# mwickert/scikit-dsp-comm

Hardware: AMD Instinct MI355X
Metric: complex64 MSamples/s (FIR-1024 tap, 2^26 samples) (higher is better)
Workload: dtype c64

## Files before the change

scikit-dsp-comm_amd/csrc/fir_ols.hip:

```cpp
#include "skdsp_internal.hpp"
#include "ols_tables.hpp"
#include "fir_route.hpp"
#include <cstdlib>
#include <cstdio>


namespace skdsp {

using namespace ols;
typedef float v4f_t __attribute__((ext_vector_type(4)));

struct OlsPlan {
    int ntaps = 0;
    int ov = 0;
    int V = 0;
    float4 *T1 = nullptr, *T2 = nullptr, *Hp = nullptr;
};

struct OlsArgs {
    const cf *x;
    cf *y;
    int64_t n, n_hist;
    const float4 *T1, *T2, *Hp;
    int ov, V, a0;
    int keep;
    int aligned;
    int64_t ntiles;
    int dec;
    unsigned dec_magic;
    int up;
    int64_t up_pitch;
    int up_sb, up_pbs, up_pb0;
    int64_t n_keep;
    const unsigned *halo_flag;
// ... 421 lines not shown
        if (DEC) {
            const unsigned j0 = r0 + (unsigned)(i + pos) * (unsigned)A.up, j1 = j0 + 64u * (unsigned)A.up;
            auto keep = [&](unsigned j, float val, bool inside) __attribute__((always_inline)) {
                const unsigned k = (unsigned)(((unsigned long long)j * A.dec_magic) >> 32);
                if (k * M == j && (int)k < qlim && inside) yq[k] = val;
            };
            keep(j0, e0.x, whole || i < lim);
            keep(j1, e1.x, whole || i + 64 < lim);
            keep(j0 + jv, e0.y, whole || i < limb);
            keep(j1 + jv, e1.y, whole || i + 64 < limb);
            continue;
        }
        char *ua = ua0 + (size_t)(a - a0) * step, *ub = ub0 + (size_t)(a - a0) * step;
        if (whole || i < lim) *reinterpret_cast<float *>(ua + b0) = e0.x;
        if (whole || i + 64 < lim) *reinterpret_cast<float *>(ua + b1) = e1.x;
        if (whole || i < limb) *reinterpret_cast<float *>(ub + b0) = e0.y;
        if (whole || i + 64 < limb) *reinterpret_cast<float *>(ub + b1) = e1.y;
    }
}


__device__ __forceinline__ OlsCareful ols_careful_args(const OlsArgs &A, int ph, bool cx)
{
    OlsCareful c;
    c.x = A.x; c.y = A.y; c.n = A.n; c.n_hist = A.n_hist; c.n_keep = A.n_keep; c.up_pitch = A.up_pitch;
    c.V = A.V; c.dec = A.dec; c.up = A.up;
    const int esz = cx ? 8 : 4;
    c.L = A.up_sb / esz;
    c.p0 = (A.up_pb0 + ph * A.up_pbs) / esz;
    c.cf = A.cf;
    return c;
}

template <bool REAL, bool DEC, bool UP = false, bool XR = false>
__global__ __launch_bounds__(256, 2) void ols_tile_kernel(OlsArgs A)
{
    __shared__ float4 lds[kLdsUnits];
    __shared__ float4 t2lds[2 * kT2Units];
    __shared__ unsigned long long ols_noted;
    if (threadIdx.x == 0) ols_noted = 0;
    constexpr int HS = (DEC && !UP) ? (REAL ? 4 : 5) : 0;
    float4 *T2f = t2lds;
    float4 *T2t = t2lds + kT2Units;
    const int t = threadIdx.x;

    {
        const float4 w = A.T2[t];
        T2f[t] = w;
        T2t[(t & 15) * 16 + (t >> 4)] = w;
    }
    cf tw[16];
#pragma unroll
    for (int k1 = 1; k1 < 16; ++k1) tw[k1] = lo(A.T1[k1 * 256 + t]);
    tw[0] = make_float2(1.f, 0.f);

    __syncthreads();
    int it = 0;
    float4 hh[16];
    int64_t tile = (gridDim.x % 8 == 0) ? (int64_t)(blockIdx.x % 8) * (gridDim.x / 8) + blockIdx.x / 8
                                                                 : (int64_t)blockIdx.x;
    const bool t0_last = A.halo_flag != nullptr;
    auto phys = [&](int64_t w) -> int64_t {
        if (UP) return (int64_t)__builtin_amdgcn_readfirstlane((unsigned)w / (unsigned)A.up);
        return t0_last ? (w + 1 < A.ntiles ? w + 1 : 0) : w;
    };
    auto phase_of = [&](int64_t w) -> int { return (int)__builtin_amdgcn_readfirstlane((unsigned)w % (unsigned)A.up); };
    if (!UP) load_H(t, A.Hp, hh);
    cf v[32];
    if (tile < A.ntiles) {
        if (t0_last && phys(tile) == 0) wait_halo(A);
        load_any<REAL, XR>(A, phys(tile), t, v);
    }
    if constexpr (XR) {
#pragma unroll
        for (int i = 0; i < 32; i += 8)
            asm volatile("" ::"v"(v[i].x), "v"(v[i + 1].x), "v"(v[i + 2].x), "v"(v[i + 3].x), "v"(v[i + 4].x), "v"(v[i + 5].x), "v"(v[i + 6].x), "v"(v[i + 7].x));
    } else {
#pragma unroll
    for (int i = 0; i < 32; i += 8)
        asm volatile("" ::"v"(v[i].x), "v"(v[i].y), "v"(v[i + 1].x), "v"(v[i + 1].y), "v"(v[i + 2].x), "v"(v[i + 2].y),
                     "v"(v[i + 3].x), "v"(v[i + 3].y), "v"(v[i + 4].x), "v"(v[i + 4].y), "v"(v[i + 5].x), "v"(v[i + 5].y),
                     "v"(v[i + 6].x), "v"(v[i + 6].y), "v"(v[i + 7].x), "v"(v[i + 7].y));
    }
    for (; tile < A.ntiles; tile += gridDim.x, ++it) {
        if (HS > 0) {
            int tt = t;
            asm volatile("" : "+v"(tt));
#pragma unroll
            for (int j = 16 - HS; j < 16; ++j) hh[j] = vld(reinterpret_cast<const volatile float4 *>(A.Hp) + (unsigned)(j * 256 + tt));
        }
        if (UP) {
            int tt = t;
            asm volatile("" : "+v"(tt));
            const volatile float4 *hp = reinterpret_cast<const volatile float4 *>(A.Hp) + (size_t)phase_of(tile) * 4096;
#pragma unroll
            for (int j = 0; j < 16; ++j) hh[j] = vld(hp + (unsigned)(j * 256 + tt));
        }
        if (REAL) fwd_pass1_real(t, v, tw, lds); else fwd_pass1(t, v, tw, lds);
        __syncthreads();
        cf Z[32];
        fwd_pass23(t, T2f, lds, Z);
        mul_H(hh, Z);
        const int64_t next = tile + gridDim.x;
        cf nx[32];
        __builtin_amdgcn_s_setprio(3);
        if (next < A.ntiles) {
            if (t0_last && phys(next) == 0) wait_halo(A);
            load_any<REAL, XR>(A, phys(next), t, nx);
        }
        __builtin_amdgcn_s_setprio(0);
        inv_pass32(t, T2t, lds, Z);
        __syncthreads();
        inv_pass1(t, tw, lds, v);
        if constexpr (XR) {
#pragma unroll
            for (int i = 0; i < 32; i += 8)
                asm volatile("" ::"v"(nx[i].x), "v"(nx[i + 1].x), "v"(nx[i + 2].x), "v"(nx[i + 3].x), "v"(nx[i + 4].x), "v"(nx[i + 5].x), "v"(nx[i + 6].x), "v"(nx[i + 7].x)
                             : "memory");
        } else {
#pragma unroll
        for (int i = 0; i < 32; i += 8)
            asm volatile("" ::"v"(nx[i].x), "v"(nx[i].y), "v"(nx[i + 1].x), "v"(nx[i + 1].y), "v"(nx[i + 2].x), "v"(nx[i + 2].y),
                         "v"(nx[i + 3].x), "v"(nx[i + 3].y), "v"(nx[i + 4].x), "v"(nx[i + 4].y), "v"(nx[i + 5].x), "v"(nx[i + 5].y),
                         "v"(nx[i + 6].x), "v"(nx[i + 6].y), "v"(nx[i + 7].x), "v"(nx[i + 7].y)
                         : "memory");
        }
        __builtin_amdgcn_s_setprio(3);
        if (UP) {
            if (!DEC && A.up_pitch) {
                OlsArgs B = A;
                B.y = REAL ? reinterpret_cast<cf *>(reinterpret_cast<float *>(A.y) + (int64_t)phase_of(tile) * A.up_pitch) : A.y + (int64_t)phase_of(tile) * A.up_pitch;
                store_any<REAL, false>(B, phys(tile), t, v, lds);
            } else if (REAL) {
                store_tile_real_up<DEC>(A, phys(tile), phase_of(tile), t, v);
            } else {
                store_tile_up<DEC>(A, phys(tile), phase_of(tile), t, v);
            }
        } else {
            store_any<REAL, DEC>(A, phys(tile), t, v, lds);
        }
        __builtin_amdgcn_s_setprio(0);
        if (__builtin_expect(__any(not_finite(v[31].x) | not_finite(v[31].y)), 0)) careful_note(&ols_noted, it);
#pragma unroll
        for (int i = 0; i < 32; ++i) v[i] = nx[i];
#ifdef SK_OLS_KEEP_B3
        __syncthreads();
#else
        if constexpr (REAL || DEC || UP || XR) __syncthreads();
#endif
    }
    const unsigned long long noted = careful_noted(&ols_noted);
    if (__builtin_expect(noted != 0, 0)) {
        int64_t w = (gridDim.x % 8 == 0) ? (int64_t)(blockIdx.x % 8) * (gridDim.x / 8) + blockIdx.x / 8 : (int64_t)blockIdx.x;
        for (int64_t k = 0; w < A.ntiles; w += gridDim.x, ++k)
            if (careful_step_noted(noted, k))
                careful_ols_tile<float, REAL, DEC, UP, XR>(ols_careful_args(A, UP ? phase_of(w) : 0, !(REAL || XR)), phys(w), UP ? phase_of(w) : 0, t);
    }
}


template <bool REAL, int MF>
__global__ __launch_bounds__(256, 2) void ols_fold_kernel(OlsArgs A)
{
    __shared__ float4 lds[kLdsUnits];
    __shared__ float4 t2lds[2 * kT2Units];
    __shared__ unsigned long long ols_noted;
    if (threadIdx.x == 0) ols_noted = 0;
    float4 *T2f = t2lds, *T2t = t2lds + kT2Units;
    const int t = threadIdx.x;
    {
        const float4 w = A.T2[t];
        T2f[t] = w;
        T2t[(t & 15) * 16 + (t >> 4)] = w;
    }
    cf tw[16];
#pragma unroll
    for (int k1 = 1; k1 < 16; ++k1) tw[k1] = lo(A.T1[k1 * 256 + t]);
    tw[0] = make_float2(1.f, 0.f);
    __syncthreads();
    float4 hh[16];
    auto first_tile = [&]() -> int64_t { return (gridDim.x % 8 == 0) ? (int64_t)(blockIdx.x % 8) * (gridDim.x / 8) + blockIdx.x / 8 : (int64_t)blockIdx.x; };
    int64_t tile = first_tile();
    load_H(t, A.Hp, hh);
    cf v[32];
    if (tile < A.ntiles) load_any<REAL, false>(A, tile, t, v);
#pragma unroll
    for (int i = 0; i < 32; i += 8)
        asm volatile("" ::"v"(v[i].x), "v"(v[i].y), "v"(v[i + 1].x), "v"(v[i + 1].y), "v"(v[i + 2].x), "v"(v[i + 2].y),
                     "v"(v[i + 3].x), "v"(v[i + 3].y), "v"(v[i + 4].x), "v"(v[i + 4].y), "v"(v[i + 5].x), "v"(v[i + 5].y),
                     "v"(v[i + 6].x), "v"(v[i + 6].y), "v"(v[i + 7].x), "v"(v[i + 7].y));
    constexpr int LS = MF / 2;
    const int b = t >> 4, q = t & 15;
    const bool active = q % LS == 0;
    const int j0 = (32 / MF) * b + q / LS;
    constexpr int JA = 512 / MF;
    for (int64_t step = 0; tile < A.ntiles; tile += gridDim.x, ++step) {
        if (REAL) fwd_pass1_real(t, v, tw, lds); else fwd_pass1(t, v, tw, lds);
        __syncthreads();
        cf Z[32];
        fwd_pass23(t, T2f, lds, Z);
        mul_H(hh, Z);
        const int64_t next = tile + gridDim.x;
        cf nx[32];
        __builtin_amdgcn_s_setprio(3);
        if (next < A.ntiles) load_any<REAL, false>(A, next, t, nx);
        __builtin_amdgcn_s_setprio(0);
        inv_pass32_fold<MF>(t, T2t, lds, Z);
        __syncthreads();
        cf o[16];
#pragma unroll
        for (int a = 0; a < 16; ++a) o[a] = make_float2(0.f, 0.f);
        inv_pass1_fold<MF>(t, tw, lds, o);
#pragma unroll
        for (int i = 0; i < 32; i += 8)
            asm volatile("" ::"v"(nx[i].x), "v"(nx[i].y), "v"(nx[i + 1].x), "v"(nx[i + 1].y), "v"(nx[i + 2].x), "v"(nx[i + 2].y),
                         "v"(nx[i + 3].x), "v"(nx[i + 3].y), "v"(nx[i + 4].x), "v"(nx[i + 4].y), "v"(nx[i + 5].x), "v"(nx[i + 5].y),
                         "v"(nx[i + 6].x), "v"(nx[i + 6].y), "v"(nx[i + 7].x), "v"(nx[i + 7].y)
                         : "memory");
// ... 90 lines not shown
            ScalarBase xc(A.x + e0);
#pragma unroll
            for (int a = 0; a < 16; ++a) {
                const v2f_t r = __builtin_nontemporal_load(xc.at<const v2f_t>(JA * 8 * a, off));
                in[a] = make_float2(r.x, r.y);
            }
        }
        return;
    }
#pragma unroll
    for (int a = 0; a < 16; ++a) {
        int64_t ia, ib;
        if (REAL) {
            const float *xr = reinterpret_cast<const float *>(A.x);
            float va = 0.f, vb = 0.f;
            if (fetch((unsigned)(JA * a + tt), ia) && ia >= -A.rep_hist && ia < A.n_in) va = xr[ia];
            if (fetch((unsigned)(JA * a + tt + VD), ib) && ib >= -A.rep_hist && ib < A.n_in) vb = xr[ib];
            in[a] = make_float2(va, vb);
        } else if (fetch((unsigned)(JA * a + tt), ia) && ia >= -A.rep_hist && ia < A.n_in) {
            in[a] = A.x[ia];
        }
    }
}

template <bool REAL, int LF>
__global__ __launch_bounds__(256, 2) void ols_rep_kernel(OlsArgs A)
{
    __shared__ float4 lds[kLdsUnits];
    __shared__ float4 t2lds[2 * kT2Units];
    __shared__ unsigned long long ols_noted;
    if (threadIdx.x == 0) ols_noted = 0;
    float4 *T2f = t2lds, *T2t = t2lds + kT2Units;
    const int t = threadIdx.x;
    {
        const float4 w = A.T2[t];
        T2f[t] = w;
        T2t[(t & 15) * 16 + (t >> 4)] = w;
    }
    cf tw[16];
#pragma unroll
    for (int k1 = 1; k1 < 16; ++k1) tw[k1] = lo(A.T1[k1 * 256 + t]);
    tw[0] = make_float2(1.f, 0.f);
    __syncthreads();
    float4 hh[16];
    auto first_tile = [&]() -> int64_t { return (gridDim.x % 8 == 0) ? (int64_t)(blockIdx.x % 8) * (gridDim.x / 8) + blockIdx.x / 8 : (int64_t)blockIdx.x; };
    int64_t tile = first_tile();
    load_H(t, A.Hp, hh);
    cf in[16];
    if (tile < A.ntiles) load_rep<REAL, LF>(A, tile, t, in);
#pragma unroll
    for (int i = 0; i < 16; i += 8)
        asm volatile("" ::"v"(in[i].x), "v"(in[i].y), "v"(in[i + 1].x), "v"(in[i + 1].y), "v"(in[i + 2].x), "v"(in[i + 2].y),
                     "v"(in[i + 3].x), "v"(in[i + 3].y), "v"(in[i + 4].x), "v"(in[i + 4].y), "v"(in[i + 5].x), "v"(in[i + 5].y),
                     "v"(in[i + 6].x), "v"(in[i + 6].y), "v"(in[i + 7].x), "v"(in[i + 7].y));
    for (int64_t step = 0; tile < A.ntiles; tile += gridDim.x, ++step) {
        fwd_pass1_rep<LF>(t, in, tw, lds);
        __syncthreads();
        cf Z[32];
        fwd_pass23_rep<LF>(t, T2f, lds, Z);
        mul_H(hh, Z);
        const int64_t next = tile + gridDim.x;
        cf nx[16];
        __builtin_amdgcn_s_setprio(3);
        if (next < A.ntiles) load_rep<REAL, LF>(A, next, t, nx);
        __builtin_amdgcn_s_setprio(0);
        inv_pass32(t, T2t, lds, Z);
        __syncthreads();
        cf v[32];
        inv_pass1(t, tw, lds, v);
#pragma unroll
        for (int i = 0; i < 16; i += 8)
            asm volatile("" ::"v"(nx[i].x), "v"(nx[i].y), "v"(nx[i + 1].x), "v"(nx[i + 1].y), "v"(nx[i + 2].x), "v"(nx[i + 2].y),
                         "v"(nx[i + 3].x), "v"(nx[i + 3].y), "v"(nx[i + 4].x), "v"(nx[i + 4].y), "v"(nx[i + 5].x), "v"(nx[i + 5].y),
                         "v"(nx[i + 6].x), "v"(nx[i + 6].y), "v"(nx[i + 7].x), "v"(nx[i + 7].y)
                         : "memory");
        __builtin_amdgcn_s_setprio(3);
        store_any<REAL, false>(A, tile, t, v, lds);
        __builtin_amdgcn_s_setprio(0);
        if (__builtin_expect(__any(not_finite(v[31].x) | not_finite(v[31].y)), 0)) careful_note(&ols_noted, step);
#pragma unroll
        for (int i = 0; i < 16; ++i) in[i] = nx[i];
        __syncthreads();
// ... 129 lines not shown
int fir_ols_launch(FirHandle *h, const void *x, int64_t n, int64_t n_hist, void *y, hipStream_t s, int dec, int reserve_wgs,
                   const unsigned *halo_flag, unsigned halo_seq, unsigned *halo_err, int halo_spins)
{
    note_path("fir_ols");
    if (n <= 0) return SKDSP_OK;
    if (dec > 1) n = (n / dec) * dec;
    if (n <= 0) return SKDSP_OK;
    SK_CHECK(fir_ols_supported(fir_shape_of(h)), SKDSP_ERR_UNSUPPORTED, "fir_ols: needs complex64 (or float32 with real taps) and 2..4097 taps");
    SK_CHECK(dec <= 32768, SKDSP_ERR_UNSUPPORTED, "fir_ols: decimation by %d (the decimating store takes M <= 32768)", dec);
    int rc = ensure_plan(h);
    if (rc) return rc;
    OlsPlan *p = h->ols;
    OlsArgs A;
    A.x = (const cf *)x;
    A.y = (cf *)y;
    A.n = n;
    A.n_hist = n_hist;
    A.T1 = p->T1; A.T2 = p->T2; A.Hp = p->Hp;
    A.ov = p->ov; A.V = p->V; A.a0 = p->ov / 512; A.keep = ols_keep_blocks(A.a0);
    const bool real = h->dtype == SKDSP_F32;
    A.aligned = ((((uintptr_t)x) | ((uintptr_t)y)) & (real ? 3 : 7)) == 0;
    int64_t ntiles = (n + p->V - 1) / p->V;
    if (real) ntiles = (ntiles + 1) / 2;
    SK_CHECK(ntiles < (int64_t)1 << 31, SKDSP_ERR_BADARG, "fir_ols: too many tiles");
    A.ntiles = ntiles;
    A.dec = dec > 1 ? dec : 1;
    A.dec_magic = A.dec > 1 ? (unsigned)((((unsigned long long)1 << 32) + A.dec - 1) / A.dec) : 0u;
    A.n_keep = n;
    A.up = 1; A.up_pitch = 0; A.up_sb = A.up_pbs = A.up_pb0 = 0;
    A.halo_flag = halo_flag; A.halo_seq = halo_seq; A.halo_err = halo_err; A.halo_spins = halo_spins > 0 ? halo_spins : (1 << 21);
    A.rep_L = 0; A.rep_lr = 1; A.rep_magic = 0; A.n_in = 0; A.rep_hist = 0;
    if ((rc = fir_careful(h, &A.cf))) return rc;
    SK_CHECK(!(halo_flag && real), SKDSP_ERR_UNSUPPORTED, "fir_ols: halo flag wait is for complex64 shards");
    int64_t grid = 2 * (int64_t)ctx().num_cus;
    if (reserve_wgs < 0) reserve_wgs = opt().ols_reserve;
    if (reserve_wgs > 0 && grid >= 4 * (int64_t)reserve_wgs) grid -= reserve_wgs;
    if (grid > ntiles) grid = ntiles;
    const int mf = A.dec % 16 == 0 ? 16 : (A.dec % 8 == 0 ? 8 : (A.dec % 4 == 0 ? 4 : (A.dec % 2 == 0 ? 2 : 1)));
    const bool fold = opt().fir_dn_fold && !halo_flag && mf > 1;
    if (fold) {
        const int mr = A.dec / mf;
        A.dec_magic = mr > 1 ? (unsigned)((((unsigned long long)1 << 32) + mr - 1) / mr) : 0u;
#define SK_FOLD(MF)                                                                                                  \
    if (real) hipLaunchKernelGGL((ols_fold_kernel<true, MF>), dim3((unsigned)grid), dim3(256), 0, s, A);             \
    else hipLaunchKernelGGL((ols_fold_kernel<false, MF>), dim3((unsigned)grid), dim3(256), 0, s, A)
        switch (mf) {
        case 2: SK_FOLD(2); break;
        case 4: SK_FOLD(4); break;
        case 8: SK_FOLD(8); break;
        default: SK_FOLD(16); break;
        }
#undef SK_FOLD
    } else if (A.dec > 1) {
        if (real) hipLaunchKernelGGL((ols_tile_kernel<true, true>), dim3((unsigned)grid), dim3(256), 0, s, A);
        else hipLaunchKernelGGL((ols_tile_kernel<false, true>), dim3((unsigned)grid), dim3(256), 0, s, A);
    } else {
        if (real) hipLaunchKernelGGL((ols_tile_kernel<true, false>), dim3((unsigned)grid), dim3(256), 0, s, A);
        else hipLaunchKernelGGL((ols_tile_kernel<false, false>), dim3((unsigned)grid), dim3(256), 0, s, A);
    }
    SK_HIP(hipGetLastError());
    return SKDSP_OK;
}


static int up_plan(FirHandle *h, int L, int kind, OlsPlan **out)
{
    const int key = kind == 1 ? -L : (kind == 2 ? 1000 + L : (kind == 3 ? 100000 + L : L));
    for (auto &u : h->ols_up)
        if (u.L == key) { *out = u.plan; return SKDSP_OK; }
    int rc = build_plan(h, L, out, kind);
// ... 5 lines not shown
static int up_walk(FirHandle *h, int kind, const void *x, int64_t n, int64_t n_hist, int L, void *y, hipStream_t s, int dec, int64_t rows_pitch)
{
    OlsPlan *p = nullptr;
    int rc = up_plan(h, L, kind, &p);
    if (rc) return rc;
    const bool xr = kind == 1;
    const bool real = h->dtype == SKDSP_F32 && !xr;
    const int cnt = kind == 1 ? L / 2 : (kind == 2 ? 1 : L);
    OlsArgs A;
    A.x = (const cf *)x;
    A.y = (cf *)y;
    A.n = n;
    A.n_hist = n_hist;
    A.T1 = p->T1; A.T2 = p->T2; A.Hp = p->Hp;
    A.ov = p->ov; A.V = p->V; A.a0 = p->ov / 512; A.keep = ols_keep_blocks(A.a0);
    const int esz = h->dtype == SKDSP_F32 ? 4 : 8;
    A.aligned = xr ? (((uintptr_t)x & 3) == 0 && ((uintptr_t)y & (L % 2 ? 3 : 7)) == 0) : ((((uintptr_t)x) | ((uintptr_t)y)) & (real ? 3 : 7)) == 0;
    int64_t ntiles = (n + p->V - 1) / p->V;
    if (real) ntiles = (ntiles + 1) / 2;
    ntiles *= cnt;
    SK_CHECK(ntiles < (int64_t)1 << 31, SKDSP_ERR_BADARG, "fir_ols_up: too many tiles");
    A.ntiles = ntiles;
    A.dec = dec;
    A.dec_magic = dec > 1 ? (unsigned)((((unsigned long long)1 << 32) + dec - 1) / dec) : 0u;
    A.n_keep = dec > 1 ? (n * L) / dec : n;
    A.up = cnt;
    A.up_pitch = dec > 1 ? 0 : rows_pitch;
    A.up_sb = L * esz;
    A.up_pbs = xr ? 8 : esz;
    A.up_pb0 = kind == 2 ? (L - 1) * esz : 0;
    A.halo_flag = nullptr; A.halo_seq = 0; A.halo_err = nullptr; A.halo_spins = 0;
    A.rep_L = 0; A.rep_lr = 1; A.rep_magic = 0; A.n_in = 0; A.rep_hist = 0;
    if ((rc = fir_careful(h, &A.cf))) return rc;
    int64_t grid = 2 * (int64_t)ctx().num_cus;
    const int reserve_wgs = opt().ols_reserve;
    if (reserve_wgs > 0 && grid >= 4 * (int64_t)reserve_wgs) grid -= reserve_wgs;
    if (grid > ntiles) grid = ntiles;
    if (xr) {
        if (L == 2 && A.up_pitch == 0) A.up_pitch = 1;
        hipLaunchKernelGGL((ols_tile_kernel<false, false, true, true>), dim3((unsigned)grid), dim3(256), 0, s, A);
    } else if (dec > 1) {
        if (real) hipLaunchKernelGGL((ols_tile_kernel<true, true, true>), dim3((unsigned)grid), dim3(256), 0, s, A);
        else hipLaunchKernelGGL((ols_tile_kernel<false, true, true>), dim3((unsigned)grid), dim3(256), 0, s, A);
    } else {
        if (real) hipLaunchKernelGGL((ols_tile_kernel<true, false, true>), dim3((unsigned)grid), dim3(256), 0, s, A);
        else hipLaunchKernelGGL((ols_tile_kernel<false, false, true>), dim3((unsigned)grid), dim3(256), 0, s, A);
    }
    SK_HIP(hipGetLastError());
    return SKDSP_OK;
}

int fir_ols_rep_launch(FirHandle *h, const void *x, int64_t n, int64_t n_hist, int L, void *y, hipStream_t s)
{
    note_path("fir_ols_rep");
    if (n <= 0) return SKDSP_OK;
    SK_CHECK(fir_ols_rep_supported(fir_shape_of(h), L, opt().fir_up_rep), SKDSP_ERR_UNSUPPORTED, "fir_ols_rep: needs complex64 (or float32 with real taps), an even L and 2..4097 taps");
    OlsPlan *p = nullptr;
    int rc = up_plan(h, L, 3, &p);
    if (rc) return rc;
    const bool real = h->dtype == SKDSP_F32;
    const int lf = L % 16 == 0 ? 16 : (L % 8 == 0 ? 8 : (L % 4 == 0 ? 4 : 2));
    OlsArgs A;
    A.x = (const cf *)x;
    A.y = (cf *)y;
    A.n = n * L;
    A.n_hist = n_hist * L;
    A.T1 = p->T1; A.T2 = p->T2; A.Hp = p->Hp;
    A.ov = p->ov; A.V = p->V; A.a0 = p->ov / 512; A.keep = ols_keep_blocks(A.a0);
    A.aligned = ((((uintptr_t)x) | ((uintptr_t)y)) & (real ? 3 : 7)) == 0;
    int64_t ntiles = (A.n + p->V - 1) / p->V;
    if (real) ntiles = (ntiles + 1) / 2;
    SK_CHECK(ntiles < (int64_t)1 << 31, SKDSP_ERR_BADARG, "fir_ols_rep: too many tiles");
    A.ntiles = ntiles;
    A.dec = 1; A.dec_magic = 0; A.n_keep = A.n;
    A.up = 1; A.up_pitch = 0; A.up_sb = A.up_pbs = A.up_pb0 = 0;
    A.halo_flag = nullptr; A.halo_seq = 0; A.halo_err = nullptr; A.halo_spins = 0;
    A.rep_L = L; A.rep_lr = L / lf;
    A.rep_magic = A.rep_lr > 1 ? (unsigned)((((unsigned long long)1 << 32) + A.rep_lr - 1) / A.rep_lr) : 0u;
    A.n_in = n; A.rep_hist = n_hist;
    if ((rc = fir_careful(h, &A.cf))) return rc;
    int64_t grid = 2 * (int64_t)ctx().num_cus;
    const int reserve_wgs = opt().ols_reserve;
    if (reserve_wgs > 0 && grid >= 4 * (int64_t)reserve_wgs) grid -= reserve_wgs;
    if (grid > ntiles) grid = ntiles;
#define SK_REP(LFV)                                                                                                  \
    if (real) hipLaunchKernelGGL((ols_rep_kernel<true, LFV>), dim3((unsigned)grid), dim3(256), 0, s, A);             \
    else hipLaunchKernelGGL((ols_rep_kernel<false, LFV>), dim3((unsigned)grid), dim3(256), 0, s, A)
    switch (lf) {
    case 2: SK_REP(2); break;
    case 4: SK_REP(4); break;
    case 8: SK_REP(8); break;
    default: SK_REP(16); break;
    }
#undef SK_REP
    SK_HIP(hipGetLastError());
    return SKDSP_OK;
}

int fir_ols_up_launch(FirHandle *h, const void *x, int64_t n, int64_t n_hist, int L, void *y, hipStream_t s, int dec, int64_t rows_pitch, int paired)
{
    note_path("fir_ols_up");
    if (n <= 0) return SKDSP_OK;
    SK_CHECK(dec >= 1 && dec <= 4096 && (dec == 1 || L <= 64), SKDSP_ERR_UNSUPPORTED, "fir_ols_up: L / M = %d / %d (the fused L / M store takes L <= 64, M <= 4096)", L, dec);
    SK_CHECK(fir_ols_up_supported(fir_shape_of(h), L), SKDSP_ERR_UNSUPPORTED, "fir_ols_up: needs complex64 (or float32 with real taps), 2 <= L <= 256, 2..4097 taps per phase");
    if (!paired) return up_walk(h, 0, x, n, n_hist, L, y, s, dec, rows_pitch);
    SK_CHECK(fir_ols_up_pairs(fir_shape_of(h), L, dec, (unsigned)(uintptr_t)y, opt().fir_up_pair) && (L % 2 == 0 || rows_pitch == 0), SKDSP_ERR_BADARG,
             "fir_ols_up: phases in pairs need float32, real taps, no decimation, and an 8-byte aligned destination (even L) or the strided form (odd L, 7 .. 13)");
    int rc = up_walk(h, 1, x, n, n_hist, L, y, s, 1, rows_pitch);
    if (rc || L % 2 == 0) return rc;
    return up_walk(h, 2, x, n, n_hist, L, y, s, 1, 0);
}

}
```

scikit-dsp-comm_amd/csrc/runtime.hip:

```cpp
#include "api_internal.hpp"
#include <cstdarg>
#include <cstdio>
#include <cstdlib>
#include <cstring>

namespace skdsp {

static thread_local char g_err[1024] = "";

void set_error(const char *fmt, ...)
{
    va_list ap;
    va_start(ap, fmt);
    vsnprintf(g_err, sizeof(g_err), fmt, ap);
    va_end(ap);
}

int hip_fail(hipError_t e, const char *what, const char *file, int line)
{
    set_error("HIP error %d (%s) in %s at %s:%d", (int)e, hipGetErrorString(e), what, file, line);
    (void)hipGetLastError();
    if (e == hipErrorOutOfMemory) return SKDSP_ERR_NOMEM;
    if (e == hipErrorNoDevice || e == hipErrorInvalidDevice) return SKDSP_ERR_NODEVICE;
    return SKDSP_ERR_HIP;
// ... 34 lines not shown
int async_err_check(Context &c)
{
    if (!c.async_err) return SKDSP_OK;
    volatile unsigned *w = c.async_err;
    if (w[kAsyncErrHalo]) {
        w[kAsyncErrHalo] = 0;
        opt().shard_two_launches = 1;
        set_error("fir_filter_shard: a sharded step since the last synchronisation gave up waiting for its halo inside the filter "
                  "launch (the first tile of that step is invalid); switched to the two-launch form (option shard_two_launches) -- "
                  "repeat the step on every rank");
        return SKDSP_ERR_RCCL;
    }
    if (w[kAsyncErrIirLookback]) {
        w[kAsyncErrIirLookback] = 0;
        set_error("iir: a look-back poll of a single-pass scan launched since the last synchronisation timed out (the results of "
                  "that call are invalid; option iir_two_pass = 1 selects the two-pass scan)");
        return SKDSP_ERR_HIP;
    }
    return SKDSP_OK;
}

int sync_checked()
{
    SK_HIP(hipStreamSynchronize(ctx().stream));
    return async_err_check(ctx());
}

namespace {
struct OptEntry { const char *name; int Options::*field; };
const OptEntry kOptTable[] = {
    {"device", &Options::device}, {"fir_algo", &Options::fir_algo}, {"dn_no_ols", &Options::dn_no_ols},
    {"fir_mm", &Options::fir_mm}, {"fir_bx", &Options::fir_bx}, 
    
    {"ols_reserve", &Options::ols_reserve}, {"fir_bx_t16", &Options::fir_bx_t16}, {"fir_bank_per", &Options::fir_bank_per}, {"ols_keep_overlap", &Options::ols_keep_overlap}, {"fir_dn_fold", &Options::fir_dn_fold}, {"fir_up_rep", &Options::fir_up_rep}, {"iir_seq", &Options::iir_seq}, {"psd_f32_image", &Options::psd_f32_image}, {"iir_up_jump", &Options::iir_up_jump}, {"iir_dn_t96", &Options::iir_dn_t96}, {"iir_up_lean", &Options::iir_up_lean}, {"iir_planar", &Options::iir_planar}, 
    {"iir_dn_full", &Options::iir_dn_full}, {"iir_no_mfma", &Options::iir_no_mfma}, 
    {"iir_two_pass", &Options::iir_two_pass}, {"iir_par", &Options::iir_par}, {"iir_par_v32", &Options::iir_par_v32}, {"iir_up_fused", &Options::iir_up_fused}, {"fir_up_ols_min", &Options::fir_up_ols_min}, {"fir_updn_fused", &Options::fir_updn_fused}, {"fir_up4k", &Options::fir_up4k}, {"fir_up4k_group", &Options::fir_up4k_group}, {"fir_up4k_staged", &Options::fir_up4k_staged}, {"fir_up2k", &Options::fir_up2k}, {"fir_dn4k", &Options::fir_dn4k}, {"fir_up_pair", &Options::fir_up_pair}, {"fir_up_rows_min", &Options::fir_up_rows_min}, {"iir_dn_compact", &Options::iir_dn_compact}, 
    {"shard_two_launches", &Options::shard_two_launches}, {"shard_probe", &Options::shard_probe}, {"shard_halo_state", &Options::shard_halo_state},
    {"shard_self_halo", &Options::shard_self_halo}, {"dist_force_comm", &Options::dist_force_comm},
    {"host_chunk_log2", &Options::host_chunk_log2}, {"host_pipeline", &Options::host_pipeline}, {"host_multi_slot", &Options::host_multi_slot},
};
int parse_opt(const char *name, const char *v)
{
    if (!strcmp(name, "fir_algo")) {
        if (!strcmp(v, "direct")) return SKDSP_FIR_DIRECT;
        if (!strcmp(v, "ols")) return SKDSP_FIR_OLS;
        if (!strcmp(v, "auto")) return SKDSP_FIR_AUTO;
    }
    if (!*v) return 1;
    return atoi(v);
}
Options options_from_env()
{
    Options o;
    for (const OptEntry &e : kOptTable) {
        char key[64] = "SKDSP_";
        size_t k = 6;
        for (const char *p = e.name; *p && k + 1 < sizeof(key); ++p) key[k++] = (char)toupper((unsigned char)*p);
        key[k] = 0;
        if (const char *v = getenv(key)) o.*(e.field) = parse_opt(e.name, v);
    }
    return o;
}
}

Options &opt()
{
    static Options o = options_from_env();
// ... 313 lines not shown
```

scikit-dsp-comm_amd/csrc/skdsp_internal.hpp:

```cpp
#pragma once
#include <hip/hip_runtime.h>
#include <stdint.h>
#include <string>
#include <vector>
#include <memory>
#include <mutex>
#include "../../include/skdsp.h"
#include "careful.hpp"

namespace skdsp {

void set_error(const char *fmt, ...);
int hip_fail(hipError_t e, const char *what, const char *file, int line);

#define SK_HIP(call)                                                        \
    do {                                                                    \
        hipError_t _e = (call);                                             \
        if (_e != hipSuccess) return skdsp::hip_fail(_e, #call, __FILE__, __LINE__); \
    } while (0)

#define SK_CHECK(cond, code, ...)            \
    do {                                     \
        if (!(cond)) {                       \
            skdsp::set_error(__VA_ARGS__);   \
            return (code);                   \
        }                                    \
    } while (0)

void note_path(const char *engine);

struct Options {
    int device = -1;
    int fir_algo = 0;
    int dn_no_ols = 0;
    int fir_mm = 1;
    int fir_bx = 1;
    int fir_bx_t16 = 1;
    int ols_keep_overlap = 1;
    int ols_reserve = 8;
    int iir_planar = 0;
    int iir_dn_full = 0;
    int iir_no_mfma = 0;
    int iir_two_pass = 0;
    int iir_par = 1;
    int iir_par_v32 = 1;
    int iir_up_jump = 1;
    int iir_seq = 1;
    int iir_up_lean = 1;
    int iir_dn_t96 = 1;
    int iir_dn_compact = 1;
    int fir_up_ols_min = 64;
    int fir_up_rows_min = -1;
    int fir_up_pair = 1;
    int fir_up4k = 1;
    int fir_up2k = 1;
    int fir_up_rep = 1;
    int fir_dn_fold = 1;
    int fir_dn4k = 1;
    int fir_up4k_group = 4;
    int fir_up4k_staged = 1;
    int fir_bank_per = 0;
    int fir_updn_fused = 1;
    int iir_up_fused = 1;
    int shard_two_launches = 0;
    int shard_probe = 1;
    int shard_halo_state = 0;
    int shard_self_halo = 0;
    int dist_force_comm = 0;
    int host_chunk_log2 = 22;
    int host_pipeline = 1;
    int psd_f32_image = 0;
    int host_multi_slot = 1;
// ... 57 lines not shown
    T *dev = nullptr;
    DevTable() = default;
    DevTable(const DevTable &) = delete;
    DevTable &operator=(const DevTable &) = delete;
    ~DevTable()
    {
        if (dev) (void)hipFree(dev);
    }
    int upload(const T *src, size_t count)
    {
        SK_HIP(hipMalloc((void **)&dev, count * sizeof(T)));
        SK_HIP(hipMemcpy(dev, src, count * sizeof(T), hipMemcpyHostToDevice));
        return SKDSP_OK;
    }
    int upload(const std::vector<T> &v) { return upload(v.data(), v.size()); }
};
struct TilePlan {
    int key = 0;
    virtual ~TilePlan() {}
};
typedef std::vector<std::unique_ptr<TilePlan>> TilePlans;
template <class P, class Fill> int tile_plan(TilePlans &plans, int key, P **out, Fill fill)
{
    for (auto &q : plans)
        if (q->key == key) { *out = static_cast<P *>(q.get()); return SKDSP_OK; }
    std::unique_ptr<P> p(new P());
    p->key = key;
    const int rc = fill(*p);
    if (rc) return rc;
    *out = p.get();
    plans.push_back(std::move(p));
    return SKDSP_OK;
}
inline int64_t persistent_grid(int64_t ntiles)
{
    int64_t grid = 2 * (int64_t)ctx().num_cus;
    const int reserve_wgs = opt().ols_reserve;
    if (reserve_wgs > 0 && grid >= 4 * (int64_t)reserve_wgs) grid -= reserve_wgs;
    return grid > ntiles ? ntiles : grid;
}
inline bool elem_aligned(const void *x, const void *y, int esz) { return ((((uintptr_t)x) | ((uintptr_t)y)) & (uintptr_t)(esz - 1)) == 0; }

struct OlsPlan;
struct Ols64Plan;
struct FirHandle : HandleBase {
    int ntaps = 0;
    bool taps_complex = false;
    int algo = SKDSP_FIR_AUTO;
    std::vector<double> taps_host;
    void *taps64_dev = nullptr;
    struct Poly { int L; int T; void *dev; };
    std::vector<Poly> poly;
    struct SwTab { int L, M, R; void *taps; void *rho; };
    std::vector<SwTab> sw;
    struct MmTab { int L, M, Lp, q, DS, RS, U0, K4; void *At; };
    std::vector<MmTab> mm;
    struct BxTab { int L, M, Lp, q, DS, RS, RT, U0, KB, RSP, KSP; float tap_inv = 0.0f; void *At = nullptr; };
    std::vector<BxTab> bx;
    OlsPlan *ols = nullptr;
    struct OlsUp { int L; OlsPlan *plan; };
    std::vector<OlsUp> ols_up;
    TilePlans up4k;
    TilePlans up2k;
    TilePlans dn4k;
    Ols64Plan *ols64 = nullptr;
    struct Ols64Up { int L; Ols64Plan *plan; };
    std::vector<Ols64Up> ols64_up;
    std::vector<FirHandle *> parts;
    int part_seg = 0;
    std::vector<FirHandle *> heads;
    ~FirHandle();
};
// ... 101 lines not shown
```

scikit-dsp-comm_amd/csrc/tile_walk.hpp:

```cpp
#pragma once
#include "ols_core.hpp"

namespace skdsp {
namespace walk {

using ols::cf;

__device__ __forceinline__ int64_t first_tile()
{
    return (gridDim.x % 8 == 0) ? (int64_t)(blockIdx.x % 8) * (gridDim.x / 8) + blockIdx.x / 8 : (int64_t)blockIdx.x;
}

__device__ __forceinline__ void twiddles_4k(int t, const float2 *T2, const float2 *tw, cf *T2f, cf *T2t, cf *twl)
{
    const cf w = T2[t];
    T2f[t] = w;
    T2t[(t & 15) * 16 + (t >> 4)] = w;
#pragma unroll
    for (int k = 0; k < 15; ++k) twl[k * 256 + t] = tw[k * 256 + t];
}

__device__ __forceinline__ float4 vld(const volatile float4 *p)
{
    float4 r;
    r.x = p->x; r.y = p->y; r.z = p->z; r.w = p->w;
    return r;
}
__device__ __forceinline__ void load_H(const float4 *Hp, int q, int t, float4 *hh)
{
    int tt = t;
    asm volatile("" : "+v"(tt));
    const volatile float4 *hp = reinterpret_cast<const volatile float4 *>(Hp) + (size_t)q * 2048;
#pragma unroll
    for (int k = 0; k < 8; ++k) hh[k] = vld(hp + (unsigned)(k * 256 + tt));
}

template <int N> __device__ __forceinline__ void pin(cf *v)
{
#pragma unroll
    for (int i = 0; i < N; i += 8)
        asm volatile("" : "+v"(v[i].x), "+v"(v[i].y), "+v"(v[i + 1].x), "+v"(v[i + 1].y), "+v"(v[i + 2].x), "+v"(v[i + 2].y), "+v"(v[i + 3].x), "+v"(v[i + 3].y),
                     "+v"(v[i + 4].x), "+v"(v[i + 4].y), "+v"(v[i + 5].x), "+v"(v[i + 5].y), "+v"(v[i + 6].x), "+v"(v[i + 6].y), "+v"(v[i + 7].x), "+v"(v[i + 7].y));
}
template <int N> __device__ __forceinline__ void settle(const float4 *hh)
// ... 25 lines not shown
```

Measured before the change: 298,600.

## Balance last-round OLS tiles across XCDs and overlap table prologue with first load

Replaces the fixed stride tile walk in the OLS tile kernel with a RoundWalk that keeps full rounds XCD-grouped but spreads the partial last round evenly across the eight XCDs. It also reorders the kernel prologue so the first input tile load is issued before twiddle, T2 and H table loads, letting that global latency overlap with table setup. Grid sizing is centralised into a helper with an optional slots override. This risks extra per-iteration index arithmetic and register pressure from holding tables alongside the first tile.

```diff
diff --git a/scikit-dsp-comm_amd/csrc/fir_ols.hip b/scikit-dsp-comm_amd/csrc/fir_ols.hip
--- a/scikit-dsp-comm_amd/csrc/fir_ols.hip
+++ b/scikit-dsp-comm_amd/csrc/fir_ols.hip
@@ -1,5 +1,6 @@
 #include "skdsp_internal.hpp"
 #include "ols_tables.hpp"
+#include "tile_walk.hpp"
 #include "fir_route.hpp"
 #include <cstdlib>
 #include <cstdio>
@@ -487,6 +488,33 @@
     return c;
 }
 
+template <bool WITH_H>
+__device__ __forceinline__ void ols_prologue_tables(const OlsArgs &A, int t, float4 *T2f, float4 *T2t, cf *tw, float4 *hh)
+{
+    const float4 w = A.T2[t];
+#pragma unroll
+    for (int k1 = 1; k1 < 16; ++k1) tw[k1] = lo(A.T1[k1 * 256 + t]);
+    tw[0] = make_float2(1.f, 0.f);
+    asm volatile("" ::: "memory");
+    if (WITH_H) load_H(t, A.Hp, hh);
+    asm volatile("" ::: "memory");
+    T2f[t] = w;
+    T2t[(t & 15) * 16 + (t >> 4)] = w;
+    __syncthreads();
+#pragma unroll
+    for (int k = 1; k < 16; k += 5)
+        asm volatile("" ::"v"(tw[k].x), "v"(tw[k].y), "v"(tw[k + 1].x), "v"(tw[k + 1].y), "v"(tw[k + 2].x), "v"(tw[k + 2].y), "v"(tw[k + 3].x), "v"(tw[k + 3].y),
+                     "v"(tw[k + 4].x), "v"(tw[k + 4].y));
+#ifdef SK_OLS_SETTLE_H
+    if (WITH_H) {
+#pragma unroll
+        for (int k = 0; k < 16; k += 4)
+            asm volatile("" ::"v"(hh[k].x), "v"(hh[k].y), "v"(hh[k].z), "v"(hh[k].w), "v"(hh[k + 1].x), "v"(hh[k + 1].y), "v"(hh[k + 1].z), "v"(hh[k + 1].w),
+                         "v"(hh[k + 2].x), "v"(hh[k + 2].y), "v"(hh[k + 2].z), "v"(hh[k + 2].w), "v"(hh[k + 3].x), "v"(hh[k + 3].y), "v"(hh[k + 3].z), "v"(hh[k + 3].w));
+    }
+#endif
+}
+
 template <bool REAL, bool DEC, bool UP = false, bool XR = false>
 __global__ __launch_bounds__(256, 2) void ols_tile_kernel(OlsArgs A)
 {
@@ -498,34 +526,24 @@
     float4 *T2f = t2lds;
     float4 *T2t = t2lds + kT2Units;
     const int t = threadIdx.x;
-
-    {
-        const float4 w = A.T2[t];
-        T2f[t] = w;
-        T2t[(t & 15) * 16 + (t >> 4)] = w;
-    }
-    cf tw[16];
-#pragma unroll
-    for (int k1 = 1; k1 < 16; ++k1) tw[k1] = lo(A.T1[k1 * 256 + t]);
-    tw[0] = make_float2(1.f, 0.f);
-
-    __syncthreads();
     int it = 0;
-    float4 hh[16];
-    int64_t tile = (gridDim.x % 8 == 0) ? (int64_t)(blockIdx.x % 8) * (gridDim.x / 8) + blockIdx.x / 8
-                                                                 : (int64_t)blockIdx.x;
+    const RoundWalk W = walk::round_walk(A.ntiles, !UP);
+    auto walk_next = [&](int64_t w, int r) -> int64_t { return UP ? w + gridDim.x : W.next(w, r); };
+    int64_t tile = W.first;
     const bool t0_last = A.halo_flag != nullptr;
     auto phys = [&](int64_t w) -> int64_t {
         if (UP) return (int64_t)__builtin_amdgcn_readfirstlane((unsigned)w / (unsigned)A.up);
         return t0_last ? (w + 1 < A.ntiles ? w + 1 : 0) : w;
     };
     auto phase_of = [&](int64_t w) -> int { return (int)__builtin_amdgcn_readfirstlane((unsigned)w % (unsigned)A.up); };
-    if (!UP) load_H(t, A.Hp, hh);
     cf v[32];
     if (tile < A.ntiles) {
         if (t0_last && phys(tile) == 0) wait_halo(A);
         load_any<REAL, XR>(A, phys(tile), t, v);
     }
+    float4 hh[16];
+    cf tw[16];
+    ols_prologue_tables<!UP>(A, t, T2f, T2t, tw, hh);
     if constexpr (XR) {
 #pragma unroll
         for (int i = 0; i < 32; i += 8)
@@ -537,7 +555,7 @@
                      "v"(v[i + 3].x), "v"(v[i + 3].y), "v"(v[i + 4].x), "v"(v[i + 4].y), "v"(v[i + 5].x), "v"(v[i + 5].y),
                      "v"(v[i + 6].x), "v"(v[i + 6].y), "v"(v[i + 7].x), "v"(v[i + 7].y));
     }
-    for (; tile < A.ntiles; tile += gridDim.x, ++it) {
+    for (; tile < A.ntiles; ++it) {
         if (HS > 0) {
             int tt = t;
             asm volatile("" : "+v"(tt));
@@ -556,7 +574,7 @@
         cf Z[32];
         fwd_pass23(t, T2f, lds, Z);
         mul_H(hh, Z);
-        const int64_t next = tile + gridDim.x;
+        const int64_t next = walk_next(tile, it);
         cf nx[32];
         __builtin_amdgcn_s_setprio(3);
         if (next < A.ntiles) {
@@ -603,11 +621,12 @@
 #else
         if constexpr (REAL || DEC || UP || XR) __syncthreads();
 #endif
+        tile = next;
     }
     const unsigned long long noted = careful_noted(&ols_noted);
     if (__builtin_expect(noted != 0, 0)) {
-        int64_t w = (gridDim.x % 8 == 0) ? (int64_t)(blockIdx.x % 8) * (gridDim.x / 8) + blockIdx.x / 8 : (int64_t)blockIdx.x;
-        for (int64_t k = 0; w < A.ntiles; w += gridDim.x, ++k)
+        int64_t w = W.first;
+        for (int k = 0; w < A.ntiles; w = walk_next(w, k), ++k)
             if (careful_step_noted(noted, k))
                 careful_ols_tile<float, REAL, DEC, UP, XR>(ols_careful_args(A, UP ? phase_of(w) : 0, !(REAL || XR)), phys(w), UP ? phase_of(w) : 0, t);
     }
@@ -623,22 +642,13 @@
     if (threadIdx.x == 0) ols_noted = 0;
     float4 *T2f = t2lds, *T2t = t2lds + kT2Units;
     const int t = threadIdx.x;
-    {
-        const float4 w = A.T2[t];
-        T2f[t] = w;
-        T2t[(t & 15) * 16 + (t >> 4)] = w;
-    }
-    cf tw[16];
-#pragma unroll
-    for (int k1 = 1; k1 < 16; ++k1) tw[k1] = lo(A.T1[k1 * 256 + t]);
-    tw[0] = make_float2(1.f, 0.f);
-    __syncthreads();
-    float4 hh[16];
     auto first_tile = [&]() -> int64_t { return (gridDim.x % 8 == 0) ? (int64_t)(blockIdx.x % 8) * (gridDim.x / 8) + blockIdx.x / 8 : (int64_t)blockIdx.x; };
     int64_t tile = first_tile();
-    load_H(t, A.Hp, hh);
     cf v[32];
     if (tile < A.ntiles) load_any<REAL, false>(A, tile, t, v);
+    float4 hh[16];
+    cf tw[16];
+    ols_prologue_tables<true>(A, t, T2f, T2t, tw, hh);
 #pragma unroll
     for (int i = 0; i < 32; i += 8)
         asm volatile("" ::"v"(v[i].x), "v"(v[i].y), "v"(v[i + 1].x), "v"(v[i + 1].y), "v"(v[i + 2].x), "v"(v[i + 2].y),
@@ -795,22 +805,13 @@
     if (threadIdx.x == 0) ols_noted = 0;
     float4 *T2f = t2lds, *T2t = t2lds + kT2Units;
     const int t = threadIdx.x;
-    {
-        const float4 w = A.T2[t];
-        T2f[t] = w;
-        T2t[(t & 15) * 16 + (t >> 4)] = w;
-    }
-    cf tw[16];
-#pragma unroll
-    for (int k1 = 1; k1 < 16; ++k1) tw[k1] = lo(A.T1[k1 * 256 + t]);
-    tw[0] = make_float2(1.f, 0.f);
-    __syncthreads();
-    float4 hh[16];
     auto first_tile = [&]() -> int64_t { return (gridDim.x % 8 == 0) ? (int64_t)(blockIdx.x % 8) * (gridDim.x / 8) + blockIdx.x / 8 : (int64_t)blockIdx.x; };
     int64_t tile = first_tile();
-    load_H(t, A.Hp, hh);
     cf in[16];
     if (tile < A.ntiles) load_rep<REAL, LF>(A, tile, t, in);
+    float4 hh[16];
+    cf tw[16];
+    ols_prologue_tables<true>(A, t, T2f, T2t, tw, hh);
 #pragma unroll
     for (int i = 0; i < 16; i += 8)
         asm volatile("" ::"v"(in[i].x), "v"(in[i].y), "v"(in[i + 1].x), "v"(in[i + 1].y), "v"(in[i + 2].x), "v"(in[i + 2].y),
@@ -1006,10 +1007,7 @@
     A.rep_L = 0; A.rep_lr = 1; A.rep_magic = 0; A.n_in = 0; A.rep_hist = 0;
     if ((rc = fir_careful(h, &A.cf))) return rc;
     SK_CHECK(!(halo_flag && real), SKDSP_ERR_UNSUPPORTED, "fir_ols: halo flag wait is for complex64 shards");
-    int64_t grid = 2 * (int64_t)ctx().num_cus;
-    if (reserve_wgs < 0) reserve_wgs = opt().ols_reserve;
-    if (reserve_wgs > 0 && grid >= 4 * (int64_t)reserve_wgs) grid -= reserve_wgs;
-    if (grid > ntiles) grid = ntiles;
+    const int64_t grid = persistent_grid(ntiles, reserve_wgs);
     const int mf = A.dec % 16 == 0 ? 16 : (A.dec % 8 == 0 ? 8 : (A.dec % 4 == 0 ? 4 : (A.dec % 2 == 0 ? 2 : 1)));
     const bool fold = opt().fir_dn_fold && !halo_flag && mf > 1;
     if (fold) {
@@ -1081,10 +1079,7 @@
     A.halo_flag = nullptr; A.halo_seq = 0; A.halo_err = nullptr; A.halo_spins = 0;
     A.rep_L = 0; A.rep_lr = 1; A.rep_magic = 0; A.n_in = 0; A.rep_hist = 0;
     if ((rc = fir_careful(h, &A.cf))) return rc;
-    int64_t grid = 2 * (int64_t)ctx().num_cus;
-    const int reserve_wgs = opt().ols_reserve;
-    if (reserve_wgs > 0 && grid >= 4 * (int64_t)reserve_wgs) grid -= reserve_wgs;
-    if (grid > ntiles) grid = ntiles;
+    const int64_t grid = persistent_grid(ntiles);
     if (xr) {
         if (L == 2 && A.up_pitch == 0) A.up_pitch = 1;
         hipLaunchKernelGGL((ols_tile_kernel<false, false, true, true>), dim3((unsigned)grid), dim3(256), 0, s, A);
@@ -1128,10 +1123,7 @@
     A.rep_magic = A.rep_lr > 1 ? (unsigned)((((unsigned long long)1 << 32) + A.rep_lr - 1) / A.rep_lr) : 0u;
     A.n_in = n; A.rep_hist = n_hist;
     if ((rc = fir_careful(h, &A.cf))) return rc;
-    int64_t grid = 2 * (int64_t)ctx().num_cus;
-    const int reserve_wgs = opt().ols_reserve;
-    if (reserve_wgs > 0 && grid >= 4 * (int64_t)reserve_wgs) grid -= reserve_wgs;
-    if (grid > ntiles) grid = ntiles;
+    const int64_t grid = persistent_grid(ntiles);
 #define SK_REP(LFV)                                                                                                  \
     if (real) hipLaunchKernelGGL((ols_rep_kernel<true, LFV>), dim3((unsigned)grid), dim3(256), 0, s, A);             \
     else hipLaunchKernelGGL((ols_rep_kernel<false, LFV>), dim3((unsigned)grid), dim3(256), 0, s, A)
diff --git a/scikit-dsp-comm_amd/csrc/ols_grid.hpp b/scikit-dsp-comm_amd/csrc/ols_grid.hpp
--- /dev/null
+++ b/scikit-dsp-comm_amd/csrc/ols_grid.hpp
@@ -0,0 +1,49 @@
+#pragma once
+#include <cstdint>
+
+#if defined(__HIPCC__)
+#define SK_GRID_HD __host__ __device__ __forceinline__
+#else
+#define SK_GRID_HD inline
+#endif
+
+namespace skdsp {
+
+inline int64_t ols_grid(int64_t ntiles, int64_t slots, int64_t reserve)
+{
+    int64_t grid = slots;
+    if (reserve > 0 && grid >= 4 * reserve) grid -= reserve;
+    return grid > ntiles ? ntiles : grid;
+}
+
+struct RoundWalk {
+    int64_t first;
+    int64_t step;
+    int32_t full_rounds;
+    int32_t last;
+    int32_t end;
+    SK_GRID_HD int64_t next(int64_t w, int32_t r) const { return r + 1 < full_rounds ? w + step : (r + 1 == full_rounds ? (int64_t)last : (int64_t)end); }
+};
+SK_GRID_HD RoundWalk ols_round_walk(int64_t wg, int64_t grid, int64_t ntiles, bool spread)
+{
+    RoundWalk W;
+    W.step = grid;
+    W.end = W.last = (int32_t)ntiles;
+    const uint32_t g = (uint32_t)grid, nt = (uint32_t)ntiles, b = (uint32_t)wg;
+    if (g % 8 != 0 || !spread) {
+        W.first = g % 8 == 0 ? (int64_t)((b % 8) * (g / 8) + b / 8) : (int64_t)b;
+        W.full_rounds = INT32_MAX;
+        return W;
+    }
+    const uint32_t per = g / 8, xcd = b % 8, j = b / 8;
+    const uint32_t rounds = (nt + g - 1) / g;
+    const uint32_t full = (rounds - 1) * g, left = nt - full;
+    const uint32_t q = left / 8, rem = left % 8;
+    const uint32_t cnt = q + (xcd < rem ? 1u : 0u), start = xcd * q + (xcd < rem ? xcd : rem);
+    W.full_rounds = (int32_t)(rounds - 1);
+    if (j < cnt) W.last = (int32_t)(full + start + j);
+    W.first = rounds > 1 ? (int64_t)(xcd * per + j) : (int64_t)W.last;
+    return W;
+}
+
+}
diff --git a/scikit-dsp-comm_amd/csrc/runtime.hip b/scikit-dsp-comm_amd/csrc/runtime.hip
--- a/scikit-dsp-comm_amd/csrc/runtime.hip
+++ b/scikit-dsp-comm_amd/csrc/runtime.hip
@@ -90,7 +90,7 @@
     {"device", &Options::device}, {"fir_algo", &Options::fir_algo}, {"dn_no_ols", &Options::dn_no_ols},
     {"fir_mm", &Options::fir_mm}, {"fir_bx", &Options::fir_bx}, 
     
-    {"ols_reserve", &Options::ols_reserve}, {"fir_bx_t16", &Options::fir_bx_t16}, {"fir_bank_per", &Options::fir_bank_per}, {"ols_keep_overlap", &Options::ols_keep_overlap}, {"fir_dn_fold", &Options::fir_dn_fold}, {"fir_up_rep", &Options::fir_up_rep}, {"iir_seq", &Options::iir_seq}, {"psd_f32_image", &Options::psd_f32_image}, {"iir_up_jump", &Options::iir_up_jump}, {"iir_dn_t96", &Options::iir_dn_t96}, {"iir_up_lean", &Options::iir_up_lean}, {"iir_planar", &Options::iir_planar}, 
+    {"ols_reserve", &Options::ols_reserve}, {"ols_grid_slots", &Options::ols_grid_slots}, {"fir_bx_t16", &Options::fir_bx_t16}, {"fir_bank_per", &Options::fir_bank_per}, {"ols_keep_overlap", &Options::ols_keep_overlap}, {"fir_dn_fold", &Options::fir_dn_fold}, {"fir_up_rep", &Options::fir_up_rep}, {"iir_seq", &Options::iir_seq}, {"psd_f32_image", &Options::psd_f32_image}, {"iir_up_jump", &Options::iir_up_jump}, {"iir_dn_t96", &Options::iir_dn_t96}, {"iir_up_lean", &Options::iir_up_lean}, {"iir_planar", &Options::iir_planar}, 
     {"iir_dn_full", &Options::iir_dn_full}, {"iir_no_mfma", &Options::iir_no_mfma}, 
     {"iir_two_pass", &Options::iir_two_pass}, {"iir_par", &Options::iir_par}, {"iir_par_v32", &Options::iir_par_v32}, {"iir_up_fused", &Options::iir_up_fused}, {"fir_up_ols_min", &Options::fir_up_ols_min}, {"fir_updn_fused", &Options::fir_updn_fused}, {"fir_up4k", &Options::fir_up4k}, {"fir_up4k_group", &Options::fir_up4k_group}, {"fir_up4k_staged", &Options::fir_up4k_staged}, {"fir_up2k", &Options::fir_up2k}, {"fir_dn4k", &Options::fir_dn4k}, {"fir_up_pair", &Options::fir_up_pair}, {"fir_up_rows_min", &Options::fir_up_rows_min}, {"iir_dn_compact", &Options::iir_dn_compact}, 
     {"shard_two_launches", &Options::shard_two_launches}, {"shard_probe", &Options::shard_probe}, {"shard_halo_state", &Options::shard_halo_state},
diff --git a/scikit-dsp-comm_amd/csrc/skdsp_internal.hpp b/scikit-dsp-comm_amd/csrc/skdsp_internal.hpp
--- a/scikit-dsp-comm_amd/csrc/skdsp_internal.hpp
+++ b/scikit-dsp-comm_amd/csrc/skdsp_internal.hpp
@@ -7,6 +7,7 @@
 #include <mutex>
 #include "../../include/skdsp.h"
 #include "careful.hpp"
+#include "ols_grid.hpp"
 
 namespace skdsp {
 
@@ -38,6 +39,7 @@
     int fir_bx_t16 = 1;
     int ols_keep_overlap = 1;
     int ols_reserve = 8;
+    int ols_grid_slots = 0;
     int iir_planar = 0;
     int iir_dn_full = 0;
     int iir_no_mfma = 0;
@@ -161,12 +163,9 @@
     plans.push_back(std::move(p));
     return SKDSP_OK;
 }
-inline int64_t persistent_grid(int64_t ntiles)
+inline int64_t persistent_grid(int64_t ntiles, int reserve_wgs = -1)
 {
-    int64_t grid = 2 * (int64_t)ctx().num_cus;
-    const int reserve_wgs = opt().ols_reserve;
-    if (reserve_wgs > 0 && grid >= 4 * (int64_t)reserve_wgs) grid -= reserve_wgs;
-    return grid > ntiles ? ntiles : grid;
+    return ols_grid(ntiles, opt().ols_grid_slots > 0 ? opt().ols_grid_slots : 2 * (int64_t)ctx().num_cus, reserve_wgs < 0 ? opt().ols_reserve : reserve_wgs);
 }
 inline bool elem_aligned(const void *x, const void *y, int esz) { return ((((uintptr_t)x) | ((uintptr_t)y)) & (uintptr_t)(esz - 1)) == 0; }
 
diff --git a/scikit-dsp-comm_amd/csrc/tile_walk.hpp b/scikit-dsp-comm_amd/csrc/tile_walk.hpp
--- a/scikit-dsp-comm_amd/csrc/tile_walk.hpp
+++ b/scikit-dsp-comm_amd/csrc/tile_walk.hpp
@@ -1,5 +1,6 @@
 #pragma once
 #include "ols_core.hpp"
+#include "ols_grid.hpp"
 
 namespace skdsp {
 namespace walk {
@@ -10,6 +11,8 @@
 {
     return (gridDim.x % 8 == 0) ? (int64_t)(blockIdx.x % 8) * (gridDim.x / 8) + blockIdx.x / 8 : (int64_t)blockIdx.x;
 }
+
+__device__ __forceinline__ RoundWalk round_walk(int64_t ntiles, bool spread = true) { return ols_round_walk((int64_t)blockIdx.x, (int64_t)gridDim.x, ntiles, spread); }
 
 __device__ __forceinline__ void twiddles_4k(int t, const float2 *T2, const float2 *tw, cf *T2f, cf *T2t, cf *twl)
 {
```

Measured after the change: 301,500, median of 5. Within noise of the previous version (+1.0%).
